# ArmingLou/seed-vc

Measured on AMD Instinct MI355X. Metric: mel_frames_per_sec, higher is better.
Workload: dtype f16; 1 GPU; seed-uvit-tat-xlsr-tiny CFM 25 steps cfg 0.7 + HiFT, batch 64 x (P=430,S=430) per GPU; batch_per_gpu=64, global_batch=64, prompt_frames=430, diffusion_steps=25, vocoder_precision=fp16p8, lanes_per_gpu=2, parallelism=utterance-sharded x1, audio gather on rank 0

## Files before the change

### include/seedvc_hip.h

```cpp
#ifndef SEEDVC_HIP_H
#define SEEDVC_HIP_H

#include <stdint.h>

#ifdef __cplusplus
extern "C" {
#endif

#define SVC_ABI_VERSION 1

typedef struct svc_tensor_desc {
    const char* name;
    const float* data;
    int ndim;
    int64_t shape[4];
} svc_tensor_desc_t;

typedef struct svc_dit_config {
    int version;
    int hidden_dim, num_heads, depth, in_channels, content_dim, style_dim;
    int final_layer_type;
    int time_as_token, style_as_token, uvit_skip_connection, long_skip_connection, style_condition;
    int wn_hidden_dim, wn_num_layers, wn_kernel_size, wn_dilation_rate;
} svc_dit_config_t;

typedef struct svc_dit svc_dit_t;

int svc_dit_create(const svc_dit_config_t* cfg, const svc_tensor_desc_t* weights, int n_weights,
                   void* stream, svc_dit_t** out);
void svc_dit_destroy(svc_dit_t* m);

int svc_dit_set_microbatch(svc_dit_t* m, int utterances);

int svc_dit_set_fused_min_rows(svc_dit_t* m, long rows);
int svc_dit_fused_available(svc_dit_t* m);
int svc_dit_set_graphs(svc_dit_t* m, int on);

typedef struct svc_cfm_args {
    int B;
    int T;
    int P;
    const float* mu;
    const float* prompt;
    const float* style;
    const float* z;
    const int64_t* x_lens;
    const int64_t* prompt_lens;
    int n_timesteps;
    float temperature;
    float cfg_rate[2];
    int random_voice;
    float* out;
} svc_cfm_args_t;

int svc_cfm_sample(svc_dit_t* m, const svc_cfm_args_t* args, void* stream);

int svc_cfm_sample_seeded(svc_dit_t* m, const svc_cfm_args_t* args, const uint64_t* seeds, void* stream);
int svc_cfm_noise_draws(uint64_t seed, int C, int T, float* z, void* stream);
// ... 241 lines not shown
```

### seed-vc_amd/_lib.py

```python
import ctypes as C
import os

import torch

_HERE = os.path.dirname(os.path.abspath(__file__))
LIB_PATH = os.path.join(_HERE, "libseedvc_hip.so")

EXPORTS = [
    "svc_abi_version", "svc_last_error",
    "svc_dit_create", "svc_dit_destroy", "svc_dit_set_microbatch", "svc_dit_set_fused_min_rows", "svc_dit_fused_available", "svc_dit_set_graphs", "svc_cfm_sample", "svc_dit_forward",
    "svc_cfm_sample_seeded", "svc_cfm_noise_draws", "svc_hift_forward_seeded", "svc_hift_noise_draws",
    "svc_bigvgan_create", "svc_bigvgan_destroy", "svc_bigvgan_forward", "svc_bigvgan_forward_ragged", "svc_bigvgan_set_microbatch",
    "svc_hift_create", "svc_hift_destroy", "svc_hift_forward", "svc_hift_forward_ragged", "svc_hift_set_microbatch",
    "svc_anti_alias_act_fwd",
    "svc_ar_create", "svc_ar_destroy", "svc_ar_reset", "svc_ar_forward_generate", "svc_ar_decode_step", "svc_ar_sample", "svc_ar_generate",
    "svc_ar_set_max_batch", "svc_ar_prefill_slot", "svc_ar_decode_step_batch", "svc_ar_generate_batch",
    "svc_ar_generate_batch_seeded", "svc_ar_exp_draws", "svc_v2_assemble_cond", "svc_mel_strip_prompt",
    "svc_ar_prefill_batch", "svc_ar_set_prefill_rows", "svc_ar_prefill_passes", "svc_ar_admit", "svc_ar_run", "svc_ar_retire",
    "svc_ar_session_active",
    "svc_lr_create", "svc_lr_destroy", "svc_lr_forward", "svc_crossfade",
    "svc_chunks_gather_cond", "svc_chunks_assemble", "svc_sola_step",
    "svc_campplus_create", "svc_campplus_destroy", "svc_campplus_forward", "svc_kaldi_fbank_frames", "svc_kaldi_fbank",
    "svc_kaldi_fbank_ragged", "svc_campplus_forward_ragged",
    "svc_mel_create", "svc_mel_destroy", "svc_mel_frames", "svc_mel_forward", "svc_mel_forward_ragged", "svc_mel_min_len",
    "svc_rmvpe_create", "svc_rmvpe_destroy", "svc_rmvpe_frames", "svc_rmvpe_min_len", "svc_rmvpe_set_plane_budget", "svc_rmvpe_set_timing", "svc_rmvpe_last_timing", "svc_rmvpe_mel",
    "svc_rmvpe_salience", "svc_rmvpe_decode", "svc_rmvpe_f0", "svc_f0_adjust",
    "svc_whisper_create", "svc_whisper_destroy", "svc_whisper_n_windows", "svc_whisper_rows", "svc_whisper_set_window_group",
    "svc_whisper_set_timing", "svc_whisper_last_timing", "svc_whisper_mel", "svc_whisper_encode", "svc_whisper_content",
    "svc_prof_enable", "svc_prof_collect",
    "svc_op_linear", "svc_op_conv1d", "svc_op_conv1d_ex", "svc_op_conv1d_last_took", "svc_op_conv_transpose1d", "svc_op_attention", "svc_op_rmsnorm",
    "svc_op_layernorm",
]

# ... 72 lines not shown
                ("out_scale", C.c_float), ("act", C.c_int32), ("act_slope", C.c_float), ("c_rows", C.c_int32), ("c_off", C.c_int32),
                ("post_a", C.c_void_p), ("post_ib", C.c_void_p), ("next_p8", C.c_int32), ("bm", C.c_int32), ("force_gemm", C.c_int32),
                ("y", C.c_void_p), ("plane_hi", C.c_void_p), ("plane_lo", C.c_void_p), ("took", C.c_int32)]


_lib = None


def lib():
    global _lib
    if _lib is None:
        if not os.path.exists(LIB_PATH):
            raise ImportError(f"{LIB_PATH} is missing: run `python -c 'import __graft_entry__ as g; g.build()'` "
                              f"(hipcc --offload-arch=gfx950); there is no CPU fallback")
        l = C.CDLL(LIB_PATH)
        l.svc_last_error.restype = C.c_char_p
        if l.svc_abi_version() != 1:
            raise ImportError("libseedvc_hip.so ABI version mismatch")
        l.svc_sola_step.argtypes = [C.c_void_p, C.c_longlong, C.c_int, C.c_int, C.c_void_p, C.c_int, C.POINTER(C.c_int32),
                                    C.c_void_p, C.c_void_p, C.c_int, C.c_int, C.c_int, C.c_void_p, C.c_void_p, C.c_void_p]
        l.svc_hift_forward_ragged.argtypes = [C.c_void_p, C.c_void_p, C.POINTER(C.c_int32), C.c_void_p, C.c_void_p, C.c_void_p,
                                              C.c_int, C.c_int, C.c_void_p, C.c_void_p, C.c_void_p]
        l.svc_op_conv1d_ex.argtypes = [C.POINTER(Conv1dEx), C.c_void_p]
        l.svc_cfm_sample_seeded.argtypes = [C.c_void_p, C.POINTER(CfmArgs), C.POINTER(C.c_uint64), C.c_void_p]
        l.svc_cfm_noise_draws.argtypes = [C.c_uint64, C.c_int, C.c_int, C.c_void_p, C.c_void_p]
        l.svc_hift_forward_seeded.argtypes = [C.c_void_p, C.c_void_p, C.POINTER(C.c_int32), C.c_void_p, C.POINTER(C.c_uint64),
                                              C.c_int, C.c_int, C.c_void_p, C.c_void_p, C.c_void_p]
        l.svc_hift_noise_draws.argtypes = [C.c_uint64, C.c_int, C.c_long, C.c_void_p, C.c_void_p, C.c_void_p]
        l.svc_mel_forward_ragged.argtypes = [C.c_void_p, C.c_void_p, C.POINTER(C.c_int32), C.c_int, C.c_int, C.c_float, C.c_void_p,
                                             C.c_void_p]
        l.svc_kaldi_fbank_ragged.argtypes = [C.c_void_p, C.c_void_p, C.POINTER(C.c_int32), C.c_int, C.c_int, C.c_int, C.c_void_p,
                                             C.c_void_p]
        l.svc_campplus_forward_ragged.argtypes = [C.c_void_p, C.c_void_p, C.POINTER(C.c_int32), C.c_int, C.c_int, C.c_void_p, C.c_void_p]
        i32p = C.POINTER(C.c_int32)
        l.svc_rmvpe_create.argtypes = [C.POINTER(RmvpeConfig), C.c_void_p, C.c_int, C.c_void_p, C.c_void_p, C.POINTER(C.c_void_p)]
        l.svc_rmvpe_set_plane_budget.argtypes = [C.c_void_p, C.c_longlong]
        l.svc_rmvpe_set_timing.argtypes = [C.c_void_p, C.c_int]
        l.svc_rmvpe_last_timing.argtypes = [C.c_void_p, C.POINTER(C.c_float)]
        l.svc_rmvpe_mel.argtypes = [C.c_void_p, C.c_void_p, i32p, C.c_int, C.c_int, C.c_void_p, C.c_void_p]
        l.svc_rmvpe_salience.argtypes = [C.c_void_p, C.c_void_p, i32p, C.c_int, C.c_int, C.c_void_p, C.c_void_p]
        l.svc_rmvpe_decode.argtypes = [C.c_void_p, i32p, C.c_int, C.c_int, C.c_float, C.c_void_p, C.c_void_p]
        l.svc_rmvpe_f0.argtypes = [C.c_void_p, C.c_void_p, i32p, C.c_int, C.c_int, C.c_float, C.c_void_p, C.c_void_p]
        l.svc_f0_adjust.argtypes = [C.c_void_p, i32p, C.c_void_p, i32p, C.c_int, C.c_int, C.c_int, C.c_int, C.POINTER(C.c_float),
                                    C.c_void_p, C.c_void_p, C.c_void_p]
        l.svc_whisper_create.argtypes = [C.POINTER(WhisperConfig), C.c_void_p, C.c_int, C.c_void_p, C.c_void_p, C.POINTER(C.c_void_p)]
        l.svc_whisper_destroy.argtypes = [C.c_void_p]
# ... 83 lines not shown
```

### seed-vc_amd/csrc/common.h

```cpp
#pragma once
#include <atomic>
#include <hip/hip_runtime.h>
#include <stdint.h>
#include <stdio.h>
#include <string>

namespace svc {

typedef _Float16 half_t;
typedef _Float16 half8 __attribute__((ext_vector_type(8)));
typedef _Float16 half4 __attribute__((ext_vector_type(4)));
typedef _Float16 half2v __attribute__((ext_vector_type(2)));
typedef float float4v __attribute__((ext_vector_type(4)));
typedef unsigned int u32x4 __attribute__((ext_vector_type(4)));

void set_error(const std::string& msg);
const char* get_error();

#define SVC_CHECK_HIP(expr)                                                                  \
    do {                                                                                     \
        hipError_t _e = (expr);                                                              \
        if (_e != hipSuccess) {                                                              \
            svc::set_error(std::string(#expr) + ": " + hipGetErrorString(_e) + " at " + __FILE__ + \
                           ":" + std::to_string(__LINE__));                                  \
// ... 141 lines not shown
    int act; float act_slope;
    const void* zero_page;
    int w8_exp;
    int c16_lo_fmt;
    const int* seq_len;
    int bm;
    int* took;
};
bool kconv_enabled();
int kconv_launch(const KConvParams& p, hipStream_t st);
__device__ __forceinline__ unsigned lo_pair_p8(float hi_as_float, float lo) {
    const float a = __builtin_amdgcn_fmed3f(hi_as_float, -448.f, 448.f), b = __builtin_amdgcn_fmed3f(lo * 2048.f, -448.f, 448.f);
    return (unsigned)__builtin_amdgcn_cvt_pk_fp8_f32(a, b, 0, false) & 0xffffu;
}
int kconv_pack_p8(const float* src, unsigned short* dst, int n0, int n1, int n2, long s0, long s1, long s2, long d0, long d1, long d2,
                  const float* scale, int* exp_out, hipStream_t st);

struct PanelParams {
    int M;
    int Lout, seq_rows, row_off;
    const half_t* wstream;
    int n_slots;
    float eps;
    int do_post;
    const half_t* ao;
    float* x;
    const float* gate_a; const float* gate_f;
    const float* g_ffn; const float* w_f; const float* b_f; int add_one;
    int I;
    half_t* c16;
    int do_skip;
    const half_t* skip_in; const float* bskip;
    int do_qkv;
    const float* g_attn; const float* w_a; const float* b_a;
    const float* rope; float q_scale;
    half_t* qk; half_t* vt; long vt_seq_stride; long vt_ld; int vt_mode;
    int do_final;
    const float* g_fin; const float* w_fin; const float* b_fin; half_t* n16;
};
bool fused_supported(int D, int I);
long fused_stream_halfs(int D, int I, bool post, bool skip, bool qkv);
long fused_pack_stream(half_t* dst, int D, int I, const float* wo, const float* w1, const float* w3, const float* w2,
                       const float* wskip, const float* wqkv, hipStream_t st);
int fused_panel_launch(const PanelParams& p, int D, bool gated, hipStream_t st);

struct AttnParams {
    const half_t* q; const half_t* k; long ld_qk;
    const half_t* vt; long vt_seq_stride; long vt_ld;
    half_t* out; long ld_out;
    int n_seq, H, seq_rows, Tq;
    int q_start;
    const int* kv_len; int kv_len_const;
    int vt_perm;
    int qt_form;
    float* out32;
};
__host__ __device__ inline int vt_perm_pos(int pos) {
    return (pos & ~31) | (((pos >> 2) & 3) << 3) | (((pos >> 4) & 1) << 2) | (pos & 3);
}
__host__ __device__ inline int vt_perm_pos16(int pos) {
    return (pos & ~12) | ((pos & 4) << 1) | ((pos & 8) >> 1);
}
// ... 15 lines not shown
```

### seed-vc_amd/csrc/dit.hip

```cpp
#include <math.h>
#include <string.h>

#include <algorithm>
#include <vector>

#include "model_util.h"
#include "noise.h"

using namespace svc;

namespace {
constexpr int MAX_STREAMS = 3;
constexpr int ROPE_POS = 8192;

float bf16_round(float f) {
    uint32_t u;
    memcpy(&u, &f, 4);
    u = (u + 0x7FFF + ((u >> 16) & 1)) & 0xFFFF0000u;
    memcpy(&f, &u, 4);
    return f;
}

std::vector<float> linspace01(int n) {
    std::vector<float> v(n);
// ... 13 lines not shown
        std::vector<float> key;
        hipGraphExec_t exec = nullptr;
        int seen = 0;
    };
    std::vector<StepGraph> graphs;
    hipStream_t cap_stream = nullptr;
    int use_graphs = 0;
    void drop_graphs() {
        for (auto& g : graphs) if (g.exec) (void)hipGraphExecDestroy(g.exec);
        graphs.clear();
    }
    PinnedRing staging;
    hipStream_t create_stream;
    int device = -1;

    struct Layer {
        half_t *wqkv, *wo, *w13, *w2, *wskip;
        float *bskip, *g_attn, *g_ffn;
        half_t* stream = nullptr;
        int stream_slots = 0;
    };
    half_t* stream_pre = nullptr;
    int stream_pre_slots = 0;
    bool fused_ok = false;
    long fused_min_rows = 10240;
    std::vector<Layer> layers;
    float* g_final;
    std::vector<int> emit, recv;
    float *te_w0, *te_b0, *te_w2, *te_b2, *te_freqs;
    float *te2_w0, *te2_b0, *te2_w2, *te2_b2, *te2_freqs;
    float *mod_w, *mod_b;
    int mod_n;
    int mod_layer_n;
    half_t* w_merge_x;
    float* w_stat;
    float* stat_const;
    float* w_style_merge;
    float *style_in_w, *style_in_b;
    half_t *head_wa, *head_w2;
    float *head_b0, *head_b2;
    half_t *w_longskip, *w_conv1, *w_resproj, *w_fl, *w_conv2;
    float *b_longskip, *b_conv1, *b_resproj, *b_fl, *b_conv2;
    float *wn_cond_w, *wn_cond_b, *fl_mod_w, *fl_mod_b;
    std::vector<half_t*> wn_in, wn_res, wn_skip;
    std::vector<float*> wn_res_b, wn_skip_b;
    half_t* wn_tail = nullptr;
// ... 102 lines not shown
        auto W = [&](const std::string& k) { return sd.get(k)->data; };
        const int slot_halfs = (D / 16) * 512;
        for (int i = 0; i < L; ++i) {
            const std::string p = "transformer.layers." + std::to_string(i) + ".";
            const bool last = i == L - 1;
            const bool nskip = !last && layers[i + 1].wskip != nullptr;
            const std::string pn = "transformer.layers." + std::to_string(i + 1) + ".";
            const long halfs = fused_stream_halfs(D, I, true, nskip, !last);
            layers[i].stream = wts.alloc_n<half_t>(halfs, st);
            if (!layers[i].stream) return 1;
            const long wr = fused_pack_stream(layers[i].stream, D, I, W(p + "attention.wo.weight"), W(p + "feed_forward.w1.weight"),
                                              W(p + "feed_forward.w3.weight"), W(p + "feed_forward.w2.weight"),
                                              nskip ? W(pn + "skip_in_linear.weight") : nullptr,
                                              last ? nullptr : W(pn + "attention.wqkv.weight"), st);
            if (wr != halfs) { set_error("fused stream packing failed"); return 1; }
            layers[i].stream_slots = (int)(halfs / slot_halfs);
        }
        const long halfs = fused_stream_halfs(D, I, false, false, true);
        stream_pre = wts.alloc_n<half_t>(halfs, st);
        if (!stream_pre) return 1;
        if (fused_pack_stream(stream_pre, D, I, nullptr, nullptr, nullptr, nullptr, nullptr,
                              W("transformer.layers.0.attention.wqkv.weight"), st) != halfs) { set_error("fused stream packing failed"); return 1; }
        stream_pre_slots = (int)(halfs / slot_halfs);
    }
    mod_layer_n = adaptive_blocks ? (v2 ? 6 * D : 4 * D) : 0;
    mod_n = L * mod_layer_n + 2 * D;
    mod_w = wts.alloc_n<float>((long)mod_n * D, st);
    mod_b = wts.alloc_n<float>(mod_n, st);
    if (!mod_w || !mod_b) return 1;
    auto put_mod = [&](const std::string& wname, const std::string& bname, int rows, long row0) -> int {
        GETW(w, wname, rows, D);
        GETW(b, bname, rows);
        if (pack_f32_launch(w->data, mod_w + row0 * D, rows, 1, D, D, 0, 1, D, 0, 1, nullptr, st)) return 1;
        SVC_CHECK_HIP(hipMemcpyAsync(mod_b + row0, b->data, rows * sizeof(float), hipMemcpyDeviceToDevice, st));
        return 0;
    };
    for (int i = 0; i < L && adaptive_blocks; ++i) {
        const std::string p = "transformer.layers." + std::to_string(i) + ".";
        if (v2) {
            if (put_mod(p + "attention_norm.linear.weight", p + "attention_norm.linear.bias", 6 * D, (long)i * mod_layer_n)) return 1;
        } else {
            if (put_mod(p + "attention_norm.project_layer.weight", p + "attention_norm.project_layer.bias", 2 * D, (long)i * mod_layer_n)) return 1;
            if (put_mod(p + "ffn_norm.project_layer.weight", p + "ffn_norm.project_layer.bias", 2 * D, (long)i * mod_layer_n + 2 * D)) return 1;
        }
    }
    if (v2) {
// ... 259 lines not shown
        xr16 = ws.alloc_n<half_t>(M * D, st);
        wnx32 = ws.alloc_n<float>(M * W, st);
        wnx16 = ws.alloc_n<half_t>(M * W, st);
        acts_stride = M * W;
        acts16 = ws.alloc_n<half_t>((long)NL * acts_stride, st);
        flin32 = ws.alloc_n<float>(M * W, st);
        fl16 = ws.alloc_n<half_t>(M * W, st);
        fo16 = ws.alloc_n<half_t>(M * W, st);
        if (!xr16 || !wnx32 || !wnx16 || !acts16 || !flin32 || !fl16 || !fo16) return 1;
    }
    d_kvlen = ws.alloc_n<int>(nseq, st);
    d_convlen = ws.alloc_n<int>(nseq, st);
    d_convlen_w = ws.alloc_n<int>(nseq, st);
    d_plen = ws.alloc_n<int>(cap_B, st);
    d_seeds = ws.alloc_n<unsigned long long>(cap_B, st);
    const long Sx = cap_steps;
    d_tvals = ws.alloc_n<float>(Sx, st);
    d_tfeat = ws.alloc_n<float>(Sx * 256, st);
    d_th = ws.alloc_n<float>(Sx * std::max(D, W), st);
    d_t1 = ws.alloc_n<float>(Sx * D, st);
    d_t1s = ws.alloc_n<float>(Sx * D, st);
    d_t2 = ws.alloc_n<float>(Sx * std::max(W, 1), st);
    d_mod = ws.alloc_n<float>(Sx * mod_n, st);
    d_gcond = ws.alloc_n<float>(Sx * std::max(2L * W * NL, 1L), st);
    d_flmod = ws.alloc_n<float>(Sx * std::max(2 * W, 1), st);
    d_stylevec = ws.alloc_n<float>((long)cap_B * D, st);
    if (!d_kvlen || !d_convlen || !d_convlen_w || !d_plen || !d_seeds || !d_tvals || !d_tfeat || !d_th || !d_t1 || !d_t1s || !d_t2 || !d_mod ||
        !d_gcond || !d_flmod || !d_stylevec)
        return 1;
    seq_rows = (int)round_up(T + npre, 8);
    vt_ld = (int)round_up(seq_rows, 64);
    SVC_CHECK_HIP(hipStreamSynchronize(st));
    return 0;
}

int svc_dit::tables(const std::vector<float>& tvals, hipStream_t st) {
    const int n = (int)tvals.size();
    {
        float* h = reinterpret_cast<float*>(staging.acquire(n * sizeof(float)));
        if (!h) return 1;
        memcpy(h, tvals.data(), n * sizeof(float));
        SVC_CHECK_HIP(hipMemcpyAsync(d_tvals, h, n * sizeof(float), hipMemcpyHostToDevice, st));
        if (staging.commit(st)) return 1;
    }
    if (timestep_feat_launch(d_tvals, te_freqs, d_tfeat, n, st)) return 1;
    if (small_linear_launch(d_tfeat, 256, te_w0, 256, te_b0, d_th, D, n, D, 256, KG_ACT_SILU, st)) return 1;
    if (small_linear_launch(d_th, D, te_w2, D, te_b2, d_t1, D, n, D, D, KG_ACT_NONE, st)) return 1;
    if (silu_launch(d_t1, d_t1s, (long)n * D, st)) return 1;
    if (small_linear_launch(v2 ? d_t1s : d_t1, D, mod_w, D, mod_b, d_mod, mod_n, n, mod_n, D, KG_ACT_NONE, st)) return 1;
    if (wavenet) {
        if (small_linear_launch(d_tfeat, 256, te2_w0, 256, te2_b0, d_th, W, n, W, 256, KG_ACT_SILU, st)) return 1;
        if (small_linear_launch(d_th, W, te2_w2, W, te2_b2, d_t2, W, n, W, W, KG_ACT_NONE, st)) return 1;
        if (small_linear_launch(d_t2, W, wn_cond_w, W, wn_cond_b, d_gcond, 2L * W * NL, n, 2 * W * NL, W, KG_ACT_NONE, st)) return 1;
        if (small_linear_launch(d_t1s, D, fl_mod_w, W, fl_mod_b, d_flmod, 2 * W, n, 2 * W, W, KG_ACT_NONE, st)) return 1;
    }
    return 0;
}


namespace {
KGemmParams gemm_base(int M, int N, int Lout) {
    KGemmParams p;
    memset(&p, 0, sizeof(p));
    p.M = M;
    p.N = N;
    p.Lout = Lout;
    p.a_seq_rows = Lout;
    p.c_seq_rows = Lout;
    p.a_stride = 1;
    p.a_len = Lout;
    p.n_taps = 1;
    p.vec_ok = 1;
// ... 211 lines not shown
        const float* fm = d_flmod + (long)step * 2 * W;
        if (layernorm_mod_launch(flin32, W, fl16, W, fm + W, fm, M, W, 1e-6f, st)) return 1;
    }
    {
        KGemmParams p = gemm_win(W);
        p.a_ptr[0] = fl16; p.a_ld[0] = W; p.a_ktiles[0] = W / 64;
        p.w = w_fl; p.ldw = W; p.bias = b_fl;
        p.c16 = fo16; p.ldc16 = W;
        if (kgemm_launch(p, 0, KG_EPI_STORE, st)) return 1;
    }
    {
        KGemmParams p = gemm_win(C);
        p.a_ptr[0] = fo16; p.a_ld[0] = W; p.a_ktiles[0] = W / 64;
        p.w = w_conv2; p.ldw = W; p.bias = b_conv2;
        p.c32 = v32; p.ldc32 = C16;
        if (kgemm_launch(p, 0, KG_EPI_STORE, st)) return 1;
    }
    return 0;
}

int svc_dit::body_fused(int n_streams, int B, int T, int step, hipStream_t st) {
    const int nseq = n_streams * B;
    const int M = nseq * seq_rows;
    const float* mod = d_mod + (long)step * mod_n;
    auto mods = [&](int i, const float** w_a, const float** b_a, const float** gate_a, const float** w_f, const float** b_f,
                    const float** gate_f) {
        *w_a = *b_a = *gate_a = *w_f = *b_f = *gate_f = nullptr;
        if (!adaptive_blocks) return;
        const float* lmod = mod + (long)i * mod_layer_n;
        if (v2) {
            *b_a = lmod; *w_a = lmod + D; *gate_a = lmod + 2 * D;
            *b_f = lmod + 3 * D; *w_f = lmod + 4 * D; *gate_f = lmod + 5 * D;
        } else {
            *w_a = lmod; *b_a = lmod + D; *w_f = lmod + 2 * D; *b_f = lmod + 3 * D;
        }
    };
    auto base = [&]() {
        PanelParams p;
        memset(&p, 0, sizeof(p));
        p.M = M; p.Lout = seq_rows; p.seq_rows = seq_rows; p.row_off = 0;
        p.eps = 1e-5f; p.add_one = v2 ? 1 : 0; p.I = I; p.x = xin;
        return p;
    };
    auto set_qkv = [&](PanelParams& p, int layer) {
        const float *w_a, *b_a, *ga, *w_f, *b_f, *gf;
        mods(layer, &w_a, &b_a, &ga, &w_f, &b_f, &gf);
        p.do_qkv = 1;
        p.g_attn = layers[layer].g_attn; p.w_a = w_a; p.b_a = b_a;
        p.rope = rope; p.q_scale = 0.125f * 1.4426950408889634f;
        p.qk = qk16; p.vt = vt; p.vt_seq_stride = (long)D * vt_ld; p.vt_ld = vt_ld; p.vt_mode = attention_vt_mode(nseq, H, seq_rows);
    };
    {
        PanelParams p = base();
        p.wstream = stream_pre; p.n_slots = stream_pre_slots;
        set_qkv(p, 0);
        if (fused_panel_launch(p, D, v2, st)) return 1;
    }
    size_t emit_i = 0;
    std::vector<int> skip_stack;
    for (int i = 0; i < L; ++i) {
        const bool last = i == L - 1;
        const bool tail_only = last && win0 > 0;
        {
            AttnParams a;
            memset(&a, 0, sizeof(a));
            a.q = qk16; a.k = qk16 + D; a.ld_qk = 2 * D;
            a.vt = vt; a.vt_seq_stride = (long)D * vt_ld; a.vt_ld = vt_ld; a.vt_perm = attention_vt_mode(nseq, H, seq_rows);
            a.out = ao16; a.ld_out = D;
            a.n_seq = nseq; a.H = H; a.seq_rows = seq_rows; a.Tq = seq_rows;
            a.q_start = tail_only ? win0 : 0;
            a.kv_len = d_kvlen;
            if (attention_launch(a, st)) return 1;
        }
        PanelParams p = base();
        const float *w_a, *b_a, *ga, *w_f, *b_f, *gf;
        mods(i, &w_a, &b_a, &ga, &w_f, &b_f, &gf);
        p.wstream = layers[i].stream; p.n_slots = layers[i].stream_slots;
        p.do_post = 1; p.ao = ao16;
        p.gate_a = ga; p.gate_f = gf; p.g_ffn = layers[i].g_ffn; p.w_f = w_f; p.b_f = b_f;
        if (std::find(emit.begin(), emit.end(), i) != emit.end()) {
            p.c16 = skip16[emit_i];
            skip_stack.push_back((int)emit_i);
            ++emit_i;
        }
        if (!last) {
            if (layers[i + 1].wskip) {
                p.do_skip = 1;
                p.skip_in = skip16[skip_stack.back()];
                skip_stack.pop_back();
                p.bskip = layers[i + 1].bskip;
            }
            set_qkv(p, i + 1);
        } else {
            const float* fm = mod + (long)L * mod_layer_n;
            p.do_final = 1; p.g_fin = g_final; p.w_fin = fm; p.b_fin = fm + D; p.n16 = n16;
            if (tail_only) { p.Lout = seq_rows - win0; p.row_off = win0; p.M = nseq * p.Lout; }
        }
        if (fused_panel_launch(p, D, v2, st)) return 1;
    }
    return 0;
}

int svc_dit::statics(int n_streams, const int (*flags)[3], int B, int T, const float* mu, const float* style_dev,
                     hipStream_t st) {
    const long Ks = C32 + Dc;
    if (w_style_merge)
        if (small_linear_launch(style_dev, S, w_style_merge, S, nullptr, d_stylevec, D, B, D, S, KG_ACT_NONE, st)) return 1;
    for (int j = 0; j < n_streams; ++j) {
        const bool use_p = flags[j][0], use_s = flags[j][1], use_m = flags[j][2];
        float* u = u_rowvec + (long)j * B * D;
        if (add_rowvec_launch(u, (use_s && w_style_merge) ? d_stylevec : nullptr, D, stat_const, B, D, st)) return 1;
        float* dst = st_term + (long)j * B * seq_rows * D;
        {
            KGemmParams p = gemm_base(B * T, D, T);
            p.a_ptr[0] = mu; p.a_ld[0] = Dc; p.a_ktiles[0] = use_m ? Dc / 32 : 0;
            p.a_seq_rows = T; p.a_len = T;
            p.w = w_stat + C32; p.ldw = Ks;
            p.c_seq_rows = seq_rows; p.c_off = npre;
// ... 259 lines not shown

void svc_dit_destroy(svc_dit_t* m) {
    if (m) {
        m->drop_graphs();
        if (m->cap_stream) (void)hipStreamDestroy(m->cap_stream);
    }
    delete m;
}

int svc_dit_set_microbatch(svc_dit_t* m, int utterances) {
    SVC_REQUIRE(m && utterances >= 0, "bad argument");
    m->microbatch = utterances;
    return 0;
}

int svc_dit_set_fused_min_rows(svc_dit_t* m, long rows) {
    SVC_REQUIRE(m, "null argument");
    m->fused_min_rows = rows < 0 ? 10240 : rows;
    return 0;
}

int svc_dit_fused_available(svc_dit_t* m) { return m && m->fused_ok ? 1 : 0; }

int svc_dit_set_graphs(svc_dit_t* m, int on) {
    SVC_REQUIRE(m, "null argument");
    m->use_graphs = on ? 1 : 0;
    if (!on) m->drop_graphs();
    return 0;
}

int svc_cfm_sample(svc_dit_t* m, const svc_cfm_args_t* a, void* stream) {
    SVC_REQUIRE(m && a, "null argument");
    return m->sample(a, nullptr, (hipStream_t)stream);
}

int svc_cfm_sample_seeded(svc_dit_t* m, const svc_cfm_args_t* a, const uint64_t* seeds, void* stream) {
    SVC_REQUIRE(m && a, "null argument");
    SVC_REQUIRE(seeds, "svc_cfm_sample_seeded: seeds is NULL (HOST [B], one per utterance)");
    return m->sample(a, seeds, (hipStream_t)stream);
}

}

int svc_dit::sample(const svc_cfm_args_t* a, const uint64_t* seeds, hipStream_t st) {
    svc_dit* m = this;
    SVC_REQUIRE(a->B >= 1 && a->T >= 1 && a->P >= 0 && a->P <= a->T && a->n_timesteps >= 1, "bad sampler shape");
// ... 91 lines not shown
```

### seed-vc_amd/csrc/fused.hip

```cpp
#include <stdlib.h>

#include <utility>

#include "common.h"

namespace svc {

namespace {

typedef __attribute__((address_space(1))) const void* gptr_t;
typedef __attribute__((address_space(3))) void* lptr_t;

template <int D>
struct PG {
    static constexpr int NT = D / 16;
    static constexpr int KC = D / 32;
    static constexpr int SLOT_BYTES = NT * 1024;
    static constexpr int NS = D == 384 ? 5 : 4;
    static constexpr int RING = NS * SLOT_BYTES;
    static constexpr int PF = D == 384 ? 6 : 4;
    static constexpr int NVEC = 9;
    static constexpr int LDS = RING + NVEC * D * 4;
};

__device__ __forceinline__ half8 frag_read(unsigned lds_addr, int off) {
    half8 r;
    asm volatile("ds_read_b128 %0, %1 offset:%2" : "=v"(r) : "v"(lds_addr), "n"(0) : "memory");
    (void)off;
    return r;
}
template <int OFF>
__device__ __forceinline__ void frag_read_to(half8& r, unsigned lds_addr) {
    asm volatile("ds_read_b128 %0, %1 offset:%2" : "=v"(r) : "v"(lds_addr), "n"(OFF));
}
template <int N>
__device__ __forceinline__ void frag_wait(half8& r) {
    asm volatile("s_waitcnt lgkmcnt(%1)" : "+v"(r) : "n"(N));
}

template <int NF, int PF, int TM, int RFI, typename F, typename R>
__device__ __forceinline__ void stream_frags(const char* base, F&& body, R&& refill) {
    static_assert(NF * 1024 <= 65536 && PF >= 1 && PF <= 8, "ds_read offset field");
    const unsigned la = (unsigned)(uintptr_t)(lptr_t)const_cast<char*>(base);
    half8 q[PF];
    [&]<int... I>(std::integer_sequence<int, I...>) { (frag_read_to<I * 1024>(q[I], la), ...); }(std::make_integer_sequence<int, PF>{});
// ... 35 lines not shown
#pragma unroll
        for (int i = 0; i < 4; ++i) body(g * 4 + i, q[g & 1][i]);
        refill(g);
        __builtin_amdgcn_sched_barrier(0);
    }
}

enum { V_AF = 0, V_BF = 1, V_GA = 2, V_GF = 3, V_AA = 4, V_BA = 5, V_BS = 6, V_AN = 7, V_BN = 8 };

template <int D, bool GATED, int TM>
__global__ __launch_bounds__(128 / (16 * TM) * 64, 128 / (16 * TM) / 4) void dit_panel_kernel(const PanelParams p) {
    using G = PG<D>;
    constexpr int NT = G::NT, KC = G::KC, NS = G::NS, PF = G::PF;
    constexpr int NW = 128 / (16 * TM), NTHR = NW * 64, DPS = NT / NW, RFI = NT / DPS;
    constexpr bool ASM_SIDE = D == 512 && TM == 2;
    extern __shared__ __attribute__((aligned(16))) char smem[];
    float* vec = reinterpret_cast<float*>(smem + G::RING);

    const int tid = threadIdx.x, lane = tid & 63;
    const int wave = __builtin_amdgcn_readfirstlane(tid >> 6);
    const int fr = lane & 15, fq = lane >> 4;
    const int m0 = blockIdx.x * 128 + wave * (16 * TM);

    for (int c = tid; c < D; c += NTHR) {
        const float one = p.add_one ? 1.f : 0.f;
        vec[V_AF * D + c] = p.g_ffn ? p.g_ffn[c] * (p.w_f ? one + p.w_f[c] : 1.f) : 0.f;
        vec[V_BF * D + c] = p.b_f ? p.b_f[c] : 0.f;
        vec[V_GA * D + c] = p.gate_a ? p.gate_a[c] : 1.f;
        vec[V_GF * D + c] = p.gate_f ? p.gate_f[c] : 1.f;
        vec[V_AA * D + c] = p.g_attn ? p.g_attn[c] * (p.w_a ? one + p.w_a[c] : 1.f) : 0.f;
        vec[V_BA * D + c] = p.b_a ? p.b_a[c] : 0.f;
        vec[V_BS * D + c] = p.bskip ? p.bskip[c] : 0.f;
        vec[V_AN * D + c] = p.g_fin ? p.g_fin[c] * (p.w_fin ? one + p.w_fin[c] : 1.f) : 0.f;
        vec[V_BN * D + c] = p.b_fin ? p.b_fin[c] : 0.f;
    }
    __syncthreads();

    const char* wsrc = reinterpret_cast<const char*>(p.wstream) + wave * (G::SLOT_BYTES / NW) + lane * 16;
    int s_next = 0, stage = 0, fill = NS - 1, s_issued = 0;
    auto piece = [&](const char* src, char* dst, int i) {
        const char* s4 = src + (i >> 2) * 4096;
        char* d4 = dst + (i >> 2) * 4096;
        switch (i & 3) {
            case 0: __builtin_amdgcn_global_load_lds((gptr_t)s4, (lptr_t)d4, 16, 0, 0); break;
            case 1: __builtin_amdgcn_global_load_lds((gptr_t)s4, (lptr_t)d4, 16, 1024, 0); break;
            case 2: __builtin_amdgcn_global_load_lds((gptr_t)s4, (lptr_t)d4, 16, 2048, 0); break;
            default: __builtin_amdgcn_global_load_lds((gptr_t)s4, (lptr_t)d4, 16, 3072, 0); break;
        }
    };
    const char* rf_src = nullptr;
    char* rf_dst = nullptr;
    auto acquire = [&]() -> const char* {
        const int ahead = p.n_slots - 1 - s_next;
        if constexpr (NS == 5) {
            if (ahead >= 3) asm volatile("s_waitcnt vmcnt(%0)" ::"n"(3 * DPS) : "memory");
            else if (ahead == 2) asm volatile("s_waitcnt vmcnt(%0)" ::"n"(2 * DPS) : "memory");
            else if (ahead == 1) asm volatile("s_waitcnt vmcnt(%0)" ::"n"(DPS) : "memory");
            else asm volatile("s_waitcnt vmcnt(0)" ::: "memory");
        } else {
            if (ahead >= 2) asm volatile("s_waitcnt vmcnt(%0)" ::"n"(2 * DPS) : "memory");
            else if (ahead == 1) asm volatile("s_waitcnt vmcnt(%0)" ::"n"(DPS) : "memory");
            else asm volatile("s_waitcnt vmcnt(0)" ::: "memory");
        }
        asm volatile("s_barrier" ::: "memory");
        const int src_slot = s_issued < p.n_slots ? s_issued : p.n_slots - 1;
        rf_src = wsrc + (long)src_slot * G::SLOT_BYTES;
        rf_dst = smem + fill * G::SLOT_BYTES + wave * (G::SLOT_BYTES / NW);
        ++s_issued;
        const char* ptr = smem + stage * G::SLOT_BYTES + lane * 16;
        stage = stage + 1 == NS ? 0 : stage + 1;
        fill = fill + 1 == NS ? 0 : fill + 1;
        ++s_next;
        return ptr;
    };
    auto refill = [&](int i) { piece(rf_src, rf_dst, i); };
#define FRAG(base, idx) (*reinterpret_cast<const half8*>((base) + (idx) * 1024))
#define MFMA(a, b, c) __builtin_amdgcn_mfma_f32_16x16x32_f16((a), (b), (c), 0, 0, 0)

#pragma unroll
    for (int s_ = 0; s_ < NS - 1; ++s_) {
        const int src_slot = s_ < p.n_slots ? s_ : p.n_slots - 1;
#pragma unroll
        for (int i = 0; i < DPS; ++i)
            piece(wsrc + (long)src_slot * G::SLOT_BYTES, smem + s_ * G::SLOT_BYTES + wave * (G::SLOT_BYTES / NW), i);
        ++s_issued;
    }

    long grow[TM];
    bool rok[TM];
#pragma unroll
    for (int mt = 0; mt < TM; ++mt) {
        const int m = m0 + 16 * mt + fr;
        rok[mt] = m < p.M;
        const int mm = rok[mt] ? m : p.M - 1;
        const int seq = mm / p.Lout;
        grow[mt] = (long)seq * p.seq_rows + p.row_off + (mm - seq * p.Lout);
    }

    float4v acc[NT][TM];
    half8 xn[KC][TM];

    auto norm_to_xn = [&](const float* va, const float* vb) {
        float rs[TM];
#pragma unroll
        for (int mt = 0; mt < TM; ++mt) {
            float ss = 0.f;
#pragma unroll
            for (int t = 0; t < NT; ++t)
#pragma unroll
// ... 22 lines not shown
    };
    auto store_x = [&]() {
#pragma unroll
        for (int mt = 0; mt < TM; ++mt)
            if (rok[mt]) {
#pragma unroll
                for (int t = 0; t < NT; ++t) *reinterpret_cast<float4v*>(p.x + grow[mt] * D + 16 * t + 4 * fq) = acc[t][mt];
            }
    };

    if (p.do_post) {
        {
            half8 af[KC][TM];
#pragma unroll
            for (int mt = 0; mt < TM; ++mt) {
#pragma unroll
                for (int kc = 0; kc < KC; ++kc)
                    af[kc][mt] = *reinterpret_cast<const half8*>(p.ao + grow[mt] * D + 32 * kc + 8 * fq);
#pragma unroll
                for (int t = 0; t < NT; ++t)
                    acc[t][mt] = GATED ? (float4v){0.f, 0.f, 0.f, 0.f}
                                       : *reinterpret_cast<const float4v*>(p.x + grow[mt] * D + 16 * t + 4 * fq);
            }
#pragma unroll
            for (int kc = 0; kc < KC; ++kc) {
                const char* base = acquire();
                stream_frags<NT, PF, TM, RFI>(base, [&](int t, half8 w) {
#pragma unroll
                    for (int mt = 0; mt < TM; ++mt) acc[t][mt] = MFMA(w, af[kc][mt], acc[t][mt]);
                }, refill);
            }
        }
        if constexpr (GATED) {
#pragma unroll
            for (int mt = 0; mt < TM; ++mt)
#pragma unroll
                for (int t = 0; t < NT; ++t) {
                    const float4v xi = *reinterpret_cast<const float4v*>(p.x + grow[mt] * D + 16 * t + 4 * fq);
                    const float4v ga = *reinterpret_cast<const float4v*>(vec + V_GA * D + 16 * t + 4 * fq);
#pragma unroll
                    for (int r = 0; r < 4; ++r) acc[t][mt][r] = xi[r] + ga[r] * acc[t][mt][r];
                }
            store_x();
        }
        norm_to_xn(vec + V_AF * D, vec + V_BF * D);
        if constexpr (GATED) {
// ... 61 lines not shown
                    const float4v xi = *reinterpret_cast<const float4v*>(p.x + grow[mt] * D + 16 * t + 4 * fq);
                    const float4v gf = *reinterpret_cast<const float4v*>(vec + V_GF * D + 16 * t + 4 * fq);
#pragma unroll
                    for (int r = 0; r < 4; ++r) acc[t][mt][r] = xi[r] + gf[r] * acc[t][mt][r];
                }
        }
        if (!p.do_skip) store_x();
        if (p.c16) {
#pragma unroll
            for (int mt = 0; mt < TM; ++mt)
                if (rok[mt]) {
#pragma unroll
                    for (int t = 0; t < NT; ++t) {
                        const half4 h = {(half_t)acc[t][mt][0], (half_t)acc[t][mt][1], (half_t)acc[t][mt][2], (half_t)acc[t][mt][3]};
                        *reinterpret_cast<half4*>(p.c16 + grow[mt] * D + 16 * t + 4 * fq) = h;
                    }
                }
        }
    } else {
#pragma unroll
        for (int mt = 0; mt < TM; ++mt)
#pragma unroll
            for (int t = 0; t < NT; ++t) acc[t][mt] = *reinterpret_cast<const float4v*>(p.x + grow[mt] * D + 16 * t + 4 * fq);
    }

    if (p.do_skip) {
#pragma unroll
        for (int c = 0; c < KC; ++c)
#pragma unroll
            for (int mt = 0; mt < TM; ++mt) {
                half8 h;
#pragma unroll
                for (int j = 0; j < 4; ++j) {
                    h[j] = (half_t)acc[2 * c][mt][j];
                    h[4 + j] = (half_t)acc[2 * c + 1][mt][j];
                }
                xn[c][mt] = h;
            }
#pragma unroll
        for (int t = 0; t < NT; ++t)
#pragma unroll
            for (int mt = 0; mt < TM; ++mt) acc[t][mt] = *reinterpret_cast<const float4v*>(vec + V_BS * D + 16 * t + 4 * fq);
#pragma unroll
        for (int kc = 0; kc < KC; ++kc) {
            const char* base = acquire();
            stream_frags<NT, PF, TM, RFI>(base, [&](int t, half8 w) {
// ... 157 lines not shown
        const int c = (int)(f / per), q = (int)(f % per);
        if (q < 2 * NT) {
            const int kc = q / 4, t = q % 4;
            const int h = 32 * c + 8 * (fr >> 2) + 2 * t + ((fr & 3) >> 1);
            const float* src = (fr & 1) ? w1 : w0;
            v = src[(long)h * D + 32 * kc + kperm];
        } else {
            const int t = q - 2 * NT;
            v = w2[(long)(16 * t + fr) * I + 32 * c + knat];
        }
    } else if (mode == 2) {
        const int kc = (int)(f / NT), t = (int)(f % NT);
        const int k = kc < KC ? 32 * kc + kperm : D + 32 * (kc - KC) + knat;
        v = w0[(long)(16 * t + fr) * (2 * D) + k];
    } else {
        const int grp = (int)(f / (4 * KC)), q = (int)(f % (4 * KC));
        const int kc = q / 4, t = q % 4;
        const int n = grp < 2 * D / 64 ? 64 * grp + 16 * (fr >> 2) + 4 * t + (fr & 3) : 64 * grp + 16 * t + fr;
        v = w0[(long)n * D + 32 * kc + kperm];
    }
    dst[e] = (half_t)v;
}

}

bool fused_supported(int D, int I) {
    static const bool off = [] { const char* e = getenv("SVC_FUSED"); return e && e[0] == '0'; }();
    return !off && (D == 384 || D == 512) && I % 32 == 0;
}

static long slots_post(int D, int I) { return D / 32 + 3L * (I / 32); }
static long slots_skip(int D) { return 2L * (D / 32); }
static long slots_qkv(int D) { return 2L * (3 * D / 64); }

long fused_stream_halfs(int D, int I, bool post, bool skip, bool qkv) {
    const long slot_halfs = (long)(D / 16) * 512;
    return ((post ? slots_post(D, I) : 0) + (skip ? slots_skip(D) : 0) + (qkv ? slots_qkv(D) : 0)) * slot_halfs;
}

long fused_pack_stream(half_t* dst, int D, int I, const float* wo, const float* w1, const float* w3, const float* w2,
                       const float* wskip, const float* wqkv, hipStream_t st) {
    const long slot_halfs = (long)(D / 16) * 512;
    long off = 0;
    auto run = [&](int mode, long slots, const float* a, const float* b, const float* c) -> bool {
        const long n = slots * slot_halfs;
        hipLaunchKernelGGL(pack_stream_kernel, dim3(cdiv(n, 256)), dim3(256), 0, st, dst + off, n, mode, D, I, a, b, c);
// ... 61 lines not shown
```

Measured before the change: 132,400 mel-frames/s.

## Precompute per-step panel vectors into a table and stream them asynchronously into LDS

Measured after the change: 133,500 mel-frames/s, median of 6. No clear change (+0.8%).

```diff
diff --git a/include/seedvc_hip.h b/include/seedvc_hip.h
--- a/include/seedvc_hip.h
+++ b/include/seedvc_hip.h
@@ -34,6 +34,7 @@
 
 int svc_dit_set_fused_min_rows(svc_dit_t* m, long rows);
 int svc_dit_fused_available(svc_dit_t* m);
+int svc_dit_panel_vectors(svc_dit_t* m, int step, int launch, float* block_out, float* mod_out, int* dims, void* stream);
 int svc_dit_set_graphs(svc_dit_t* m, int on);
 
 typedef struct svc_cfm_args {
diff --git a/seed-vc_amd/_lib.py b/seed-vc_amd/_lib.py
--- a/seed-vc_amd/_lib.py
+++ b/seed-vc_amd/_lib.py
@@ -8,7 +8,7 @@
 
 EXPORTS = [
     "svc_abi_version", "svc_last_error",
-    "svc_dit_create", "svc_dit_destroy", "svc_dit_set_microbatch", "svc_dit_set_fused_min_rows", "svc_dit_fused_available", "svc_dit_set_graphs", "svc_cfm_sample", "svc_dit_forward",
+    "svc_dit_create", "svc_dit_destroy", "svc_dit_set_microbatch", "svc_dit_set_fused_min_rows", "svc_dit_fused_available", "svc_dit_panel_vectors", "svc_dit_set_graphs", "svc_cfm_sample", "svc_dit_forward",
     "svc_cfm_sample_seeded", "svc_cfm_noise_draws", "svc_hift_forward_seeded", "svc_hift_noise_draws",
     "svc_bigvgan_create", "svc_bigvgan_destroy", "svc_bigvgan_forward", "svc_bigvgan_forward_ragged", "svc_bigvgan_set_microbatch",
     "svc_hift_create", "svc_hift_destroy", "svc_hift_forward", "svc_hift_forward_ragged", "svc_hift_set_microbatch",
@@ -127,6 +127,7 @@
         l.svc_hift_forward_ragged.argtypes = [C.c_void_p, C.c_void_p, C.POINTER(C.c_int32), C.c_void_p, C.c_void_p, C.c_void_p,
                                               C.c_int, C.c_int, C.c_void_p, C.c_void_p, C.c_void_p]
         l.svc_op_conv1d_ex.argtypes = [C.POINTER(Conv1dEx), C.c_void_p]
+        l.svc_dit_panel_vectors.argtypes = [C.c_void_p, C.c_int, C.c_int, C.c_void_p, C.c_void_p, C.POINTER(C.c_int), C.c_void_p]
         l.svc_cfm_sample_seeded.argtypes = [C.c_void_p, C.POINTER(CfmArgs), C.POINTER(C.c_uint64), C.c_void_p]
         l.svc_cfm_noise_draws.argtypes = [C.c_uint64, C.c_int, C.c_int, C.c_void_p, C.c_void_p]
         l.svc_hift_forward_seeded.argtypes = [C.c_void_p, C.c_void_p, C.POINTER(C.c_int32), C.c_void_p, C.POINTER(C.c_uint64),
diff --git a/seed-vc_amd/csrc/common.h b/seed-vc_amd/csrc/common.h
--- a/seed-vc_amd/csrc/common.h
+++ b/seed-vc_amd/csrc/common.h
@@ -187,22 +187,23 @@
     const half_t* wstream;
     int n_slots;
     float eps;
+    const float* vecs;
     int do_post;
     const half_t* ao;
     float* x;
-    const float* gate_a; const float* gate_f;
-    const float* g_ffn; const float* w_f; const float* b_f; int add_one;
     int I;
     half_t* c16;
     int do_skip;
-    const half_t* skip_in; const float* bskip;
+    const half_t* skip_in;
     int do_qkv;
-    const float* g_attn; const float* w_a; const float* b_a;
     const float* rope; float q_scale;
     half_t* qk; half_t* vt; long vt_seq_stride; long vt_ld; int vt_mode;
     int do_final;
-    const float* g_fin; const float* w_fin; const float* b_fin; half_t* n16;
-};
+    half_t* n16;
+};
+long fused_vec_block_floats(int D);
+int fused_pack_vectors(float* table, int n_steps, int L, int D, const float* mod, int mod_n, int mod_layer_n, int v2,
+                       const float* lw, const float* g_final, hipStream_t st);
 bool fused_supported(int D, int I);
 long fused_stream_halfs(int D, int I, bool post, bool skip, bool qkv);
 long fused_pack_stream(half_t* dst, int D, int I, const float* wo, const float* w1, const float* w3, const float* w2,
diff --git a/seed-vc_amd/csrc/dit.hip b/seed-vc_amd/csrc/dit.hip
--- a/seed-vc_amd/csrc/dit.hip
+++ b/seed-vc_amd/csrc/dit.hip
@@ -59,6 +59,10 @@
     };
     half_t* stream_pre = nullptr;
     int stream_pre_slots = 0;
+    float* lw_vec = nullptr;
+    float* d_vecs = nullptr;
+    long vec_block = 0;
+    int vec_steps = 0;
     bool fused_ok = false;
     long fused_min_rows = 10240;
     std::vector<Layer> layers;
@@ -207,6 +211,15 @@
         if (fused_pack_stream(stream_pre, D, I, nullptr, nullptr, nullptr, nullptr, nullptr,
                               W("transformer.layers.0.attention.wqkv.weight"), st) != halfs) { set_error("fused stream packing failed"); return 1; }
         stream_pre_slots = (int)(halfs / slot_halfs);
+        vec_block = fused_vec_block_floats(D);
+        lw_vec = wts.alloc_n<float>((long)L * 3 * D, st);
+        if (!lw_vec) return 1;
+        SVC_CHECK_HIP(hipMemsetAsync(lw_vec, 0, (size_t)L * 3 * D * sizeof(float), st));
+        for (int i = 0; i < L; ++i) {
+            const float* src[3] = {layers[i].g_attn, layers[i].g_ffn, layers[i].wskip ? layers[i].bskip : nullptr};
+            for (int k = 0; k < 3; ++k)
+                if (src[k]) SVC_CHECK_HIP(hipMemcpyAsync(lw_vec + ((long)i * 3 + k) * D, src[k], D * sizeof(float), hipMemcpyDeviceToDevice, st));
+        }
     }
     mod_layer_n = adaptive_blocks ? (v2 ? 6 * D : 4 * D) : 0;
     mod_n = L * mod_layer_n + 2 * D;
@@ -512,6 +525,12 @@
     d_t1s = ws.alloc_n<float>(Sx * D, st);
     d_t2 = ws.alloc_n<float>(Sx * std::max(W, 1), st);
     d_mod = ws.alloc_n<float>(Sx * mod_n, st);
+    d_vecs = nullptr;
+    vec_steps = 0;
+    if (fused_ok) {
+        d_vecs = ws.alloc_n<float>(Sx * (L + 1) * vec_block, st);
+        if (!d_vecs) return 1;
+    }
     d_gcond = ws.alloc_n<float>(Sx * std::max(2L * W * NL, 1L), st);
     d_flmod = ws.alloc_n<float>(Sx * std::max(2 * W, 1), st);
     d_stylevec = ws.alloc_n<float>((long)cap_B * D, st);
@@ -538,6 +557,10 @@
     if (small_linear_launch(d_th, D, te_w2, D, te_b2, d_t1, D, n, D, D, KG_ACT_NONE, st)) return 1;
     if (silu_launch(d_t1, d_t1s, (long)n * D, st)) return 1;
     if (small_linear_launch(v2 ? d_t1s : d_t1, D, mod_w, D, mod_b, d_mod, mod_n, n, mod_n, D, KG_ACT_NONE, st)) return 1;
+    if (fused_ok) {
+        if (fused_pack_vectors(d_vecs, n, L, D, d_mod, mod_n, mod_layer_n, v2 ? 1 : 0, lw_vec, g_final, st)) return 1;
+        vec_steps = n;
+    }
     if (wavenet) {
         if (small_linear_launch(d_tfeat, 256, te2_w0, 256, te2_b0, d_th, W, n, W, 256, KG_ACT_SILU, st)) return 1;
         if (small_linear_launch(d_th, W, te2_w2, W, te2_b2, d_t2, W, n, W, W, KG_ACT_NONE, st)) return 1;
@@ -795,38 +818,25 @@
 int svc_dit::body_fused(int n_streams, int B, int T, int step, hipStream_t st) {
     const int nseq = n_streams * B;
     const int M = nseq * seq_rows;
-    const float* mod = d_mod + (long)step * mod_n;
-    auto mods = [&](int i, const float** w_a, const float** b_a, const float** gate_a, const float** w_f, const float** b_f,
-                    const float** gate_f) {
-        *w_a = *b_a = *gate_a = *w_f = *b_f = *gate_f = nullptr;
-        if (!adaptive_blocks) return;
-        const float* lmod = mod + (long)i * mod_layer_n;
-        if (v2) {
-            *b_a = lmod; *w_a = lmod + D; *gate_a = lmod + 2 * D;
-            *b_f = lmod + 3 * D; *w_f = lmod + 4 * D; *gate_f = lmod + 5 * D;
-        } else {
-            *w_a = lmod; *b_a = lmod + D; *w_f = lmod + 2 * D; *b_f = lmod + 3 * D;
-        }
-    };
-    auto base = [&]() {
+    SVC_REQUIRE(step < vec_steps, "fused path: the vector table does not cover this step");
+    const float* vecs = d_vecs + (long)step * (L + 1) * vec_block;
+    auto base = [&](int launch) {
         PanelParams p;
         memset(&p, 0, sizeof(p));
         p.M = M; p.Lout = seq_rows; p.seq_rows = seq_rows; p.row_off = 0;
-        p.eps = 1e-5f; p.add_one = v2 ? 1 : 0; p.I = I; p.x = xin;
+        p.eps = 1e-5f; p.I = I; p.x = xin;
+        p.vecs = vecs + (long)launch * vec_block;
         return p;
     };
-    auto set_qkv = [&](PanelParams& p, int layer) {
-        const float *w_a, *b_a, *ga, *w_f, *b_f, *gf;
-        mods(layer, &w_a, &b_a, &ga, &w_f, &b_f, &gf);
+    auto set_qkv = [&](PanelParams& p) {
         p.do_qkv = 1;
-        p.g_attn = layers[layer].g_attn; p.w_a = w_a; p.b_a = b_a;
         p.rope = rope; p.q_scale = 0.125f * 1.4426950408889634f;
         p.qk = qk16; p.vt = vt; p.vt_seq_stride = (long)D * vt_ld; p.vt_ld = vt_ld; p.vt_mode = attention_vt_mode(nseq, H, seq_rows);
     };
     {
-        PanelParams p = base();
+        PanelParams p = base(0);
         p.wstream = stream_pre; p.n_slots = stream_pre_slots;
-        set_qkv(p, 0);
+        set_qkv(p);
         if (fused_panel_launch(p, D, v2, st)) return 1;
     }
     size_t emit_i = 0;
@@ -845,12 +855,9 @@
             a.kv_len = d_kvlen;
             if (attention_launch(a, st)) return 1;
         }
-        PanelParams p = base();
-        const float *w_a, *b_a, *ga, *w_f, *b_f, *gf;
-        mods(i, &w_a, &b_a, &ga, &w_f, &b_f, &gf);
+        PanelParams p = base(i + 1);
         p.wstream = layers[i].stream; p.n_slots = layers[i].stream_slots;
         p.do_post = 1; p.ao = ao16;
-        p.gate_a = ga; p.gate_f = gf; p.g_ffn = layers[i].g_ffn; p.w_f = w_f; p.b_f = b_f;
         if (std::find(emit.begin(), emit.end(), i) != emit.end()) {
             p.c16 = skip16[emit_i];
             skip_stack.push_back((int)emit_i);
@@ -861,12 +868,10 @@
                 p.do_skip = 1;
                 p.skip_in = skip16[skip_stack.back()];
                 skip_stack.pop_back();
-                p.bskip = layers[i + 1].bskip;
             }
-            set_qkv(p, i + 1);
+            set_qkv(p);
         } else {
-            const float* fm = mod + (long)L * mod_layer_n;
-            p.do_final = 1; p.g_fin = g_final; p.w_fin = fm; p.b_fin = fm + D; p.n16 = n16;
+            p.do_final = 1; p.n16 = n16;
             if (tail_only) { p.Lout = seq_rows - win0; p.row_off = win0; p.M = nseq * p.Lout; }
         }
         if (fused_panel_launch(p, D, v2, st)) return 1;
@@ -1172,6 +1177,21 @@
 
 int svc_dit_fused_available(svc_dit_t* m) { return m && m->fused_ok ? 1 : 0; }
 
+int svc_dit_panel_vectors(svc_dit_t* m, int step, int launch, float* block_out, float* mod_out, int* dims, void* stream) {
+    SVC_REQUIRE(m && dims, "svc_dit_panel_vectors: null argument");
+    SVC_REQUIRE(m->fused_ok, "svc_dit_panel_vectors: this width has no fused kernel");
+    dims[0] = (int)m->vec_block; dims[1] = m->mod_n; dims[2] = m->L + 1; dims[3] = m->vec_steps;
+    if (!block_out && !mod_out) return 0;
+    SVC_REQUIRE(step >= 0 && step < m->vec_steps && launch >= 0 && launch <= m->L, "svc_dit_panel_vectors: no such block in the table of the last call");
+    hipStream_t st = (hipStream_t)stream;
+    if (block_out)
+        SVC_CHECK_HIP(hipMemcpyAsync(block_out, m->d_vecs + ((long)step * (m->L + 1) + launch) * m->vec_block, m->vec_block * sizeof(float),
+                                     hipMemcpyDeviceToDevice, st));
+    if (mod_out)
+        SVC_CHECK_HIP(hipMemcpyAsync(mod_out, m->d_mod + (long)step * m->mod_n, m->mod_n * sizeof(float), hipMemcpyDeviceToDevice, st));
+    return 0;
+}
+
 int svc_dit_set_graphs(svc_dit_t* m, int on) {
     SVC_REQUIRE(m, "null argument");
     m->use_graphs = on ? 1 : 0;
diff --git a/seed-vc_amd/csrc/fused.hip b/seed-vc_amd/csrc/fused.hip
--- a/seed-vc_amd/csrc/fused.hip
+++ b/seed-vc_amd/csrc/fused.hip
@@ -20,7 +20,8 @@
     static constexpr int RING = NS * SLOT_BYTES;
     static constexpr int PF = D == 384 ? 6 : 4;
     static constexpr int NVEC = 9;
-    static constexpr int LDS = RING + NVEC * D * 4;
+    static constexpr int VEC_PIECES = (NVEC * D * 4 + 1023) / 1024;
+    static constexpr int LDS = RING + VEC_PIECES * 1024;
 };
 
 __device__ __forceinline__ half8 frag_read(unsigned lds_addr, int off) {
@@ -102,20 +103,6 @@
     const int fr = lane & 15, fq = lane >> 4;
     const int m0 = blockIdx.x * 128 + wave * (16 * TM);
 
-    for (int c = tid; c < D; c += NTHR) {
-        const float one = p.add_one ? 1.f : 0.f;
-        vec[V_AF * D + c] = p.g_ffn ? p.g_ffn[c] * (p.w_f ? one + p.w_f[c] : 1.f) : 0.f;
-        vec[V_BF * D + c] = p.b_f ? p.b_f[c] : 0.f;
-        vec[V_GA * D + c] = p.gate_a ? p.gate_a[c] : 1.f;
-        vec[V_GF * D + c] = p.gate_f ? p.gate_f[c] : 1.f;
-        vec[V_AA * D + c] = p.g_attn ? p.g_attn[c] * (p.w_a ? one + p.w_a[c] : 1.f) : 0.f;
-        vec[V_BA * D + c] = p.b_a ? p.b_a[c] : 0.f;
-        vec[V_BS * D + c] = p.bskip ? p.bskip[c] : 0.f;
-        vec[V_AN * D + c] = p.g_fin ? p.g_fin[c] * (p.w_fin ? one + p.w_fin[c] : 1.f) : 0.f;
-        vec[V_BN * D + c] = p.b_fin ? p.b_fin[c] : 0.f;
-    }
-    __syncthreads();
-
     const char* wsrc = reinterpret_cast<const char*>(p.wstream) + wave * (G::SLOT_BYTES / NW) + lane * 16;
     int s_next = 0, stage = 0, fill = NS - 1, s_issued = 0;
     auto piece = [&](const char* src, char* dst, int i) {
@@ -157,14 +144,26 @@
 #define FRAG(base, idx) (*reinterpret_cast<const half8*>((base) + (idx) * 1024))
 #define MFMA(a, b, c) __builtin_amdgcn_mfma_f32_16x16x32_f16((a), (b), (c), 0, 0, 0)
 
-#pragma unroll
-    for (int s_ = 0; s_ < NS - 1; ++s_) {
-        const int src_slot = s_ < p.n_slots ? s_ : p.n_slots - 1;
-#pragma unroll
-        for (int i = 0; i < DPS; ++i)
-            piece(wsrc + (long)src_slot * G::SLOT_BYTES, smem + s_ * G::SLOT_BYTES + wave * (G::SLOT_BYTES / NW), i);
-        ++s_issued;
-    }
+    {
+        constexpr int VPW = (G::VEC_PIECES + NW - 1) / NW;
+        static_assert(VPW <= 8, "piece() immediates");
+        const char* vsrc = reinterpret_cast<const char*>(p.vecs) + wave * (VPW * 1024) + lane * 16;
+        char* vdst = smem + G::RING + wave * (VPW * 1024);
+#pragma unroll
+        for (int i = 0; i < VPW; ++i)
+            if (wave * VPW + i < G::VEC_PIECES) piece(vsrc, vdst, i);
+    }
+
+    auto prime_ring = [&]() {
+#pragma unroll
+        for (int s_ = 0; s_ < NS - 1; ++s_) {
+            const int src_slot = s_ < p.n_slots ? s_ : p.n_slots - 1;
+#pragma unroll
+            for (int i = 0; i < DPS; ++i)
+                piece(wsrc + (long)src_slot * G::SLOT_BYTES, smem + s_ * G::SLOT_BYTES + wave * (G::SLOT_BYTES / NW), i);
+            ++s_issued;
+        }
+    };
 
     long grow[TM];
     bool rok[TM];
@@ -233,6 +232,7 @@
                     acc[t][mt] = GATED ? (float4v){0.f, 0.f, 0.f, 0.f}
                                        : *reinterpret_cast<const float4v*>(p.x + grow[mt] * D + 16 * t + 4 * fq);
             }
+            prime_ring();
 #pragma unroll
             for (int kc = 0; kc < KC; ++kc) {
                 const char* base = acquire();
@@ -340,6 +340,9 @@
         for (int mt = 0; mt < TM; ++mt)
 #pragma unroll
             for (int t = 0; t < NT; ++t) acc[t][mt] = *reinterpret_cast<const float4v*>(p.x + grow[mt] * D + 16 * t + 4 * fq);
+        prime_ring();
+        asm volatile("s_waitcnt vmcnt(%0)" ::"n"((NS - 1) * DPS) : "memory");
+        asm volatile("s_barrier" ::: "memory");
     }
 
     if (p.do_skip) {
@@ -543,6 +546,50 @@
     dst[e] = (half_t)v;
 }
 
+__global__ void panel_vectors_kernel(float* __restrict__ table, int block_floats, int L, int D, const float* __restrict__ mod,
+                                     int mod_n, int mod_layer_n, int v2, const float* __restrict__ lw,
+                                     const float* __restrict__ g_final) {
+    const int j = blockIdx.x, step = blockIdx.y;
+    float* blk = table + ((long)step * (L + 1) + j) * block_floats;
+    const float* m = mod + (long)step * mod_n;
+    const bool adaptive = mod_layer_n > 0;
+    const float one = v2 ? 1.f : 0.f;
+    const float* mf = m + (long)(j - 1) * mod_layer_n;
+    const float* ma = m + (long)j * mod_layer_n;
+    const float* fm = m + (long)L * mod_layer_n;
+    const int o_wa = v2 ? D : 0, o_ba = v2 ? 0 : D, o_wf = v2 ? 4 * D : 2 * D, o_bf = 3 * D;
+    const bool post = j >= 1, pre = j < L, fin = j == L;
+    for (int e = threadIdx.x; e < block_floats; e += blockDim.x) {
+        const int v = e / D, c = e - v * D;
+        float r = 0.f;
+        switch (v) {
+            case V_AF: if (post) r = lw[((long)(j - 1) * 3 + 1) * D + c] * (adaptive ? one + mf[o_wf + c] : 1.f); break;
+            case V_BF: if (post && adaptive) r = mf[o_bf + c]; break;
+            case V_GA: r = post && adaptive && v2 ? mf[2 * D + c] : 1.f; break;
+            case V_GF: r = post && adaptive && v2 ? mf[5 * D + c] : 1.f; break;
+            case V_AA: if (pre) r = lw[((long)j * 3 + 0) * D + c] * (adaptive ? one + ma[o_wa + c] : 1.f); break;
+            case V_BA: if (pre && adaptive) r = ma[o_ba + c]; break;
+            case V_BS: if (post && pre) r = lw[((long)j * 3 + 2) * D + c]; break;
+            case V_AN: if (fin) r = g_final[c] * (one + fm[c]); break;
+            case V_BN: if (fin) r = fm[D + c]; break;
+            default: break;
+        }
+        blk[e] = r;
+    }
+}
+
+}
+
+long fused_vec_block_floats(int D) { return (long)((PG<384>::NVEC * D * 4 + 1023) / 1024) * 256; }
+
+int fused_pack_vectors(float* table, int n_steps, int L, int D, const float* mod, int mod_n, int mod_layer_n, int v2,
+                       const float* lw, const float* g_final, hipStream_t st) {
+    SVC_REQUIRE(D == 384 || D == 512, "fused vector table: D must be 384 or 512");
+    SVC_REQUIRE(table && mod && lw && g_final && n_steps >= 1 && L >= 1, "fused vector table: bad argument");
+    hipLaunchKernelGGL(panel_vectors_kernel, dim3(L + 1, n_steps), dim3(256), 0, st, table, (int)fused_vec_block_floats(D), L, D,
+                       mod, mod_n, mod_layer_n, v2, lw, g_final);
+    SVC_CHECK_HIP(hipGetLastError());
+    return 0;
 }
 
 bool fused_supported(int D, int I) {
```
